# henry-yeh/DeepACO

Measured on AMD Instinct MI355X. Metric: ant-tours/sec, TSP-500 n_ants=512, higher is better.
Workload: dtype f32; 1 GPU; TSP-500 random-Euclidean, n_ants=512, 64 instances per GPU, AS update, heuristic 1/d sparsified k=50, sampler=auto -> scan_sparse; nodes=500, n_ants=512, instances_per_gpu=64, sampler=scan_sparse, parallelism=instance-sharded x1

## Files before the change

### deepaco_amd/csrc/daco_scan_sparse.hip

```cpp
#include "daco_sample_kernel.h"
#include "daco_head_rows.h"
#include "daco_tour_epilogue.h"

namespace daco {

constexpr int SP_FCMP_OGT = 2, SP_FCMP_OGE = 3, SP_FCMP_OLT = 4;

enum : uint32_t { STREAM_SPARSE = 4, STREAM_SPARSE_RETRY = 5 };

template <int N> __device__ inline float sp_row_bcast(float x) { return dpp_f<0x150 + N, 0xF, false>(x, x); }
template <int N> __device__ inline int sp_row_ror(int x) { return dpp_i<0x120 + N, 0xF, false>(x, x); }
__device__ inline float sp_row_scan(float x) {
  x = x + dpp_f<DPP_ROW_SHR(1), 0xF, true>(0.0f, x);
  x = x + dpp_f<DPP_ROW_SHR(2), 0xF, true>(0.0f, x);
  x = x + dpp_f<DPP_ROW_SHR(4), 0xF, true>(0.0f, x);
  x = x + dpp_f<DPP_ROW_SHR(8), 0xF, true>(0.0f, x);
  return x;
}
__device__ inline uint64_t sp_row_first(uint64_t m) { return m & ~((m | 0x8000800080008000ull) - 0x0001000100010001ull); }

template <bool RACE, bool VEC4, int CH>
__global__ void __launch_bounds__(256)
sparse_prepass_kernel(int B, int n, int ch, const float *tau, long tau_bs, const float *eta, long eta_bs,
                      const uint16_t *hid, float *P, char *hrow, int spl, int dead) {
  __shared__ uint32_t bm[4][32];
  const int lane = threadIdx.x & 63, wave = threadIdx.x >> 6;
  const long row = (long)blockIdx.x * 4 + wave;
  if (row >= (long)B * n) return;
  const int b = (int)(row / n), r = (int)(row - (long)b * n);
  const float *tr = tau + b * tau_bs + (long)r * n, *er = eta + b * eta_bs + (long)r * n;
  emit_head_row<RACE, CH, VEC4>(n, ch, tr, er, hid + row * (16 * spl), bm[wave], hrow + row * sp_head_row_bytes(spl), P + row * (256 * ch), spl, dead, lane);
}

template <int CH>
__global__ void __launch_bounds__(256)
sparse_prepass_ut_kernel(int B, int n, int ch, const float *tau, long tau_bs, const float *heta, float tail_c, const uint16_t *hid,
                         char *hrow, int spl, int dead) {
  __shared__ uint32_t bm[4][32];
  const int lane = threadIdx.x & 63, wave = threadIdx.x >> 6;
  const long row = (long)blockIdx.x * 4 + wave;
  if (row >= (long)B * n) return;
  const int b = (int)(row / n), r = (int)(row - (long)b * n);
  HeadUt h;
  head_ut_fetch(h, n, heta + row * (16 * spl), hid + row * (16 * spl), spl, lane);
  emit_head_row_ut<CH>(n, ch, tau + b * tau_bs + (long)r * n, tail_c, h, bm[wave], hrow + row * sp_head_row_bytes(spl), spl, dead, lane);
}

typedef uint32_t sp_u32x4 __attribute__((ext_vector_type(4)));
typedef uint32_t sp_u32x2 __attribute__((ext_vector_type(2)));
struct SpRowSrc { const float *p; };
struct SpRowUT { __amdgpu_buffer_rsrc_t t; float c; };
struct SpRowTE { __amdgpu_buffer_rsrc_t t, e; };
__device__ __forceinline__ __amdgpu_buffer_rsrc_t sp_row_rsrc(const float *row, int n) {
  return __builtin_amdgcn_make_buffer_rsrc((void *)row, 0, (int)((uint32_t)n * 4u), 0x00020000);
}
__device__ __forceinline__ int sp_lane_off(const SpRowSrc &, int lane) { return lane; }
template <class Src> __device__ __forceinline__ int sp_lane_off(const Src &, int lane) {
  int lo = lane * 16;
  asm volatile("" : "+v"(lo));
  return lo;
}
__device__ __forceinline__ float4 sp_row4(const SpRowSrc &r, int c, int lo) { return *reinterpret_cast<const float4 *>(r.p + (c * 64 + lo) * 4); }
__device__ __forceinline__ float4 sp_row4(const SpRowUT &r, int c, int lo) {
  const sp_u32x4 t = __builtin_amdgcn_raw_buffer_load_b128(r.t, lo + c * 1024, 0, 0);
  return make_float4(__uint_as_float(t.x) * r.c, __uint_as_float(t.y) * r.c, __uint_as_float(t.z) * r.c, __uint_as_float(t.w) * r.c);
}
__device__ __forceinline__ float4 sp_row4(const SpRowTE &r, int c, int lo) {
  const sp_u32x4 t = __builtin_amdgcn_raw_buffer_load_b128(r.t, lo + c * 1024, 0, 0), e = __builtin_amdgcn_raw_buffer_load_b128(r.e, lo + c * 1024, 0, 0);
  return make_float4(__uint_as_float(t.x) * __uint_as_float(e.x), __uint_as_float(t.y) * __uint_as_float(e.y),
                     __uint_as_float(t.z) * __uint_as_float(e.z), __uint_as_float(t.w) * __uint_as_float(e.w));
}

typedef const __attribute__((address_space(4))) SampleParams *sp_args_t;
template <bool UT>
__device__ __forceinline__ auto sp_row_of(const float *base, sp_args_t pa, int b, int row, int ld, int n) {
  if constexpr (UT) asm volatile("" : "+s"(pa));
  if constexpr (UT) return SpRowUT{sp_row_rsrc(pa->tau + (size_t)b * pa->tau_bs + (size_t)row * n, n), pa->tail_c};
  else return SpRowSrc{base + (size_t)row * ld};
}

template <int CHD, bool TAIL, class Src>
__device__ __forceinline__ int sparse_row_walk(const Src &rowp, const uint8_t *flg, const uint32_t *bm, int lane, float ur) {
  constexpr int NJ = CHD * 4;
  float run[16];
  float acc = 0.0f;
  uint32_t pos = 0;
  const int lo = sp_lane_off(rowp, lane);
#pragma unroll
  for (int c = 0; c < CHD; ++c) {
    const int k0 = (c * 64 + lane) * 4;
    if constexpr (std::is_same<Src, SpRowTE>::value) __builtin_amdgcn_sched_barrier(0);
    const float4 rv = sp_row4(rowp, c, lo);
    float f[4];
    if constexpr (TAIL) {
      const uint32_t w = bm[(k0 >> 5) & 31] >> (k0 & 31);
      f[0] = (w & 1u) ? 0.0f : 1.0f; f[1] = (w & 2u) ? 0.0f : 1.0f; f[2] = (w & 4u) ? 0.0f : 1.0f; f[3] = (w & 8u) ? 0.0f : 1.0f;
    } else {
      const uint32_t ff = *reinterpret_cast<const uint32_t *>(flg + k0);
      f[0] = (float)(ff & 0xFFu); f[1] = (float)((ff >> 8) & 0xFFu); f[2] = (float)((ff >> 16) & 0xFFu); f[3] = (float)(ff >> 24);
    }
    acc = __builtin_fmaf(rv.x, f[0], acc); run[4 * c + 0] = acc;
    acc = __builtin_fmaf(rv.y, f[1], acc); run[4 * c + 1] = acc;
    acc = __builtin_fmaf(rv.z, f[2], acc); run[4 * c + 2] = acc;
    acc = __builtin_fmaf(rv.w, f[3], acc); run[4 * c + 3] = acc;
    pos |= (rv.x * f[0] > 0.0f ? 1u : 0u) << (4 * c) | (rv.y * f[1] > 0.0f ? 2u : 0u) << (4 * c) |
           (rv.z * f[2] > 0.0f ? 4u : 0u) << (4 * c) | (rv.w * f[3] > 0.0f ? 8u : 0u) << (4 * c);
  }
#pragma unroll
  for (int j = NJ; j < 16; ++j) run[j] = __builtin_inff();
  const float part = acc;
  const float incl = wave_scan_add(part);
  float r = ur;
  if constexpr (!TAIL) {
    const float S = readlane_f(incl, 63);
    if (!(S > 0.0f)) return -1;
    r = ur * S;
    r = r > 0.0f ? r : 1.401298464e-45f;
  }
  uint64_t m = __ballot(incl >= r && part > 0.0f);
  int L;
  if (m == 0) {
    if constexpr (!TAIL) return -1;
    m = __ballot(part > 0.0f);
    if (m == 0) return -1;
    L = 63 - __builtin_clzll(m);
  } else {
    L = __builtin_ctzll(m);
  }
  const float excl = L ? readlane_f(incl, L - 1) : 0.0f;
  const float thr = fmaxf(r - excl, 1.401298464e-45f);
  const int cnt = count_below<NJ>(run, thr);
  int jsel = readlane_i(cnt, L);
  if (jsel >= NJ) {
    const uint32_t pl = (uint32_t)readlane_i((int)pos, L);
    jsel = pl ? 31 - __builtin_clz(pl) : 0;
  }
  return ((jsel >> 2) * 64 + L) * 4 + (jsel & 3);
}

__device__ inline float sp_at_least_denorm(float x) {
  float y;
  asm("v_max_f32 %0, 1, %1" : "=v"(y) : "v"(x));
  return y;
}

constexpr int SP_W = 352;
constexpr int SP_EW = 160;
constexpr int SP_ST_DEAD = 16 * (512 + 16) + 4 * 128 + 256;
constexpr int SP_ST_LDS = SP_ST_DEAD + 16 * SP_W * 2;
static_assert(SP_ST_LDS <= 160 * 1024 / 8 && SP_ST_DEAD % 16 == 0, "ST: eight workgroups per CU");
static_assert(SP_ST_DEAD >= 16 * SP_EW * 2 + 4 * 512 * 2, "ST: early parts and the inverse table of four ants inside the dead bytes");

static_assert(std::is_trivially_copyable<SampleParams>::value, "SampleParams is read back from the kernel-argument segment as plain bytes");
template <int CHD, bool RACE, int SPL, bool LH = false, bool ST = false, bool UT = false>
__global__ void __launch_bounds__(256, LH ? 1 : (ST ? 8 : (CHD == 2 ? (RACE ? 4 : 6) : 5)))
scan_sparse_kernel(const SampleParams p) {
  static_assert(!UT || !RACE, "the uniform-tail mode: scan draw");
  static_assert(!LH || (CHD == 2 && !RACE && SPL == 4), "the LDS-heads variant: n <= 512, scan draw, 64-slot heads");
  static_assert(!ST || (CHD == 2 && !RACE && SPL == 4 && !LH), "the split-tour variant: n <= 512, scan draw, 64-slot heads, not LH");
  constexpr int APW = 4, APB = LH ? 4 : 16;
  constexpr int LS = sp_lane_bytes(SPL);
  constexpr int LAST = SPL - 1;
  constexpr int FL = CHD * 256;
  constexpr int FLP = FL + 16;
  constexpr int FLT = FL + 2;
  constexpr uint32_t ROWB = 16u * LS;
  constexpr bool TG = CHD == 4;
  extern __shared__ __attribute__((aligned(16))) unsigned char sparse_dyn[];
  uint8_t *flag_mem = sparse_dyn;
  uint16_t *tour_mem = reinterpret_cast<uint16_t *>(sparse_dyn + (ST ? SP_ST_DEAD : APB * FLP));
  __shared__ uint32_t bm_static[TG || ST ? 1 : (LH ? 1 : 4)][32];
  uint32_t (*bm_s)[32] = TG ? reinterpret_cast<uint32_t (*)[32]>(sparse_dyn + APB * FLP + APB * 32)
                            : ST ? reinterpret_cast<uint32_t (*)[32]>(sparse_dyn + APB * FLP) : bm_static;
  unsigned char *lh_tab = sparse_dyn + APB * FLP + APB * FLT * 2;
  static_assert(!LH || ((APB * FLP + APB * FLT * 2) % 16 == 0), "LH: table aligned");
  const int lane = threadIdx.x & 63, wave = __builtin_amdgcn_readfirstlane(threadIdx.x >> 6);
  const int q = lane >> 4, s = lane & 15;
  const int w = xcd_remap(blockIdx.x, gridDim.x);
  const int bpi = (p.A + APB - 1) / APB;
  const int b = w / bpi;
  const int abase = (w - b * bpi) * APB;
  const int a0 = abase + wave * APW;
  const int n = p.n, A = p.A;
  const uint64_t iter_now = p.iter + (p.iter_dev ? *p.iter_dev : 0ull);
  const bool active = a0 < A && (!LH || wave == 0);
  const int a = a0 + q < A ? a0 + q : A - 1;
  const uint32_t gid = p.ant_gid0 + (uint32_t)(b * (p.gid_bstride ? p.gid_bstride : A) + a);
  const float *Pb = UT ? nullptr : p.P + (size_t)b * n * p.ld;
  const char *hrb = (const char *)p.hval + (size_t)b * n * ROWB;
  const __amdgpu_buffer_rsrc_t hres = __builtin_amdgcn_make_buffer_rsrc((void *)hrb, 0, (int)((uint32_t)n * ROWB), 0x00020000);
#define SP_ROW_OF(pv) sp_row_of<UT>(Pb, (sp_args_t)__builtin_amdgcn_kernarg_segment_ptr(), b, pv, p.ld, n)
  uint32_t sls = (uint32_t)s * LS;
  asm volatile("" : "+v"(sls));
  uint8_t *fl = flag_mem + (wave * APW + q) * FLP;
  uint16_t *tour = tour_mem + (wave * APW + q) * (TG ? 16 : ST ? SP_W : FLT);
  uint16_t *t16b = TG || ST ? p.tours16 + ((size_t)b * A + abase) * FL : nullptr;
  const int TE = ST ? (n > SP_W ? (n - SP_W + 15) & ~15 : 0) : 0;
  const uint32_t t16o = (uint32_t)((wave * APW + q) * FL + s);
#define SP_T(t) (TG ? ((t) & 15) : (t))
  bool infeasible = false;
  unsigned long long n_dense = 0, n_tail = 0, n_rej = 0;
  uint32_t lh_rb = 0, lh_rbsel = 0, lh_loff = 0, lh_toff = 0;
  if constexpr (LH) {
    const int kl = p.lh_kl, kmax = p.lh_kmax;
    lh_rb = (uint32_t)kl * LS;
    lh_toff = (uint32_t)(kmax / SPL) * LS + (uint32_t)(kmax % SPL) * 4u;
    lh_rbsel = s < kl ? lh_rb : 0u;
    lh_loff = s < kl ? (uint32_t)s * LS : (uint32_t)n * lh_rb;
    const char *src = hrb;
    const int l16 = threadIdx.x & 15;
    if (l16 < kl)
      for (int row0 = threadIdx.x >> 4; row0 < n; row0 += 16 * 8) {
        uint2 x[8][3];
#pragma unroll
        for (int u = 0; u < 8; ++u) {
          const int row = row0 + 16 * u;
          const uint2 *g = reinterpret_cast<const uint2 *>(src + (size_t)(row < n ? row : row0) * ROWB + l16 * LS);
          x[u][0] = g[0]; x[u][1] = g[1]; x[u][2] = g[2];
        }
#pragma unroll
        for (int u = 0; u < 8; ++u) {
          const int row = row0 + 16 * u;
          if (row < n) {
            uint2 *d = reinterpret_cast<uint2 *>(lh_tab + (uint32_t)row * lh_rb + l16 * LS);
            d[0] = x[u][0]; d[1] = x[u][1]; d[2] = x[u][2];
          }
        }
      }
    if (threadIdx.x < 4) reinterpret_cast<float *>(lh_tab + (uint32_t)n * lh_rb)[threadIdx.x] = 0.0f;
    if (threadIdx.x >= 4 && threadIdx.x < 6) reinterpret_cast<uint32_t *>(lh_tab + (uint32_t)n * lh_rb)[threadIdx.x] = (uint32_t)p.ld * 0x00010001u;
    __syncthreads();
    bool too_many = false;
    for (int row = threadIdx.x; row < n; row += 256) {
      const char *gr = src + (size_t)row * ROWB;
      const uint16_t idk = *reinterpret_cast<const uint16_t *>(gr + (kmax / SPL) * LS + SPL * 4 + (kmax % SPL) * 2);
      too_many |= idk != (uint16_t)p.ld;
      *reinterpret_cast<float *>(lh_tab + (uint32_t)row * lh_rb + lh_toff) = *reinterpret_cast<const float *>(gr + 15 * LS + LAST * 4);
    }
    if (too_many && p.flags) atomicOr(p.flags + b, 4);
    __syncthreads();
  }

  if (active) {
    {
      const uint4 ones = make_uint4(0x01010101u, 0x01010101u, 0x01010101u, 0x01010101u);
#pragma unroll
      for (int g = 0; g < FL / 256; ++g) *(uint4 *)(fl + g * 256 + s * 16) = ones;
      fl[FL + s] = 0;
    }
    int prev;
    if (p.start) prev = (int)p.start[(size_t)b * A + a];
    else if (p.fixed_start >= 0) prev = p.fixed_start;
    else {
      const u32x4 r = rng_block(p.seed, iter_now, STREAM_START, gid, 0);
      prev = (int)__umulhi(r.x, (uint32_t)n);
    }
    __builtin_amdgcn_wave_barrier();
    if (s == 0) { fl[prev] = 0; tour[0] = (uint16_t)prev; }
    asm volatile("" ::: "memory");
    __builtin_amdgcn_wave_barrier();
    u32x4 ublk = {0, 0, 0, 0};
    float ucur = 0.0f;
    for (int t0 = 0; t0 < n; t0 += 16) {
      int t = t0;
      if constexpr (ST) {
        if (t0 == TE && t0 != 0) {
          int lf = lane;
          asm volatile("" : "+v"(lf) :: "memory");
          const int qf = lf >> 4;
          const uint4 *src = reinterpret_cast<const uint4 *>(tour);
          uint4 *dst = reinterpret_cast<uint4 *>(t16b + (size_t)(wave * APW + qf) * FL);
          for (int j = lf & 15; j < (TE >> 3); j += 16) {
            const uint4 v = src[j];
            if (a0 + qf < A) dst[j] = v;
          }
          asm volatile("" ::: "memory");
          tour -= TE;
        }
      }
      if constexpr (!RACE) {
        if ((t0 & 63) == 0) ublk = rng_block(p.seed, iter_now, STREAM_SPARSE, gid, (uint32_t)(((t0 >> 6) << 4) + (15 - s)));
        ucur = u01(comp(ublk, (t0 >> 4) & 3));
        if (t0 == 0) ucur = __int_as_float(sp_row_ror<1>(__float_as_int(ucur)));
      }
      if (t0 == 0) t = 1;
      const int te = t0 + 16 < n ? t0 + 16 : n;
#ifndef DACO_SPARSE_UNROLL
#define DACO_SPARSE_UNROLL 1
#endif
#pragma unroll DACO_SPARSE_UNROLL
      for (; t < te; ++t) {
        const uint32_t off = LH ? __umul24((uint32_t)prev, lh_rbsel) + lh_loff : __umul24((uint32_t)prev, ROWB) + sls;
        float h[SPL];
        uint32_t w0, w1, w2 = 0, w3 = 0;
        if constexpr (LH) {
          const uint2 ra = *reinterpret_cast<const uint2 *>(lh_tab + off), rb_ = *reinterpret_cast<const uint2 *>(lh_tab + off + 8),
                      rc = *reinterpret_cast<const uint2 *>(lh_tab + off + 16);
          const float tv = *reinterpret_cast<const float *>(lh_tab + __umul24((uint32_t)prev, lh_rb) + lh_toff);
          h[0] = __uint_as_float(ra.x); h[1] = __uint_as_float(ra.y); h[2] = __uint_as_float(rb_.x);
          h[3] = s == 15 ? tv : __uint_as_float(rb_.y);
          w0 = rc.x; w1 = rc.y;
        } else if constexpr (SPL == 4) {
          const sp_u32x4 hvr = __builtin_amdgcn_raw_buffer_load_b128(hres, off, 0, 0);
          const sp_u32x2 hi2 = __builtin_amdgcn_raw_buffer_load_b64(hres, off + 16u, 0, 0);
          h[0] = __uint_as_float(hvr.x); h[1] = __uint_as_float(hvr.y); h[2] = __uint_as_float(hvr.z); h[3] = __uint_as_float(hvr.w);
          w0 = hi2.x; w1 = hi2.y;
        } else {
          const sp_u32x4 hva = __builtin_amdgcn_raw_buffer_load_b128(hres, off, 0, 0);
          const sp_u32x4 hvb = __builtin_amdgcn_raw_buffer_load_b128(hres, off + 16u, 0, 0);
          const sp_u32x4 hi4 = __builtin_amdgcn_raw_buffer_load_b128(hres, off + 32u, 0, 0);
          h[0] = __uint_as_float(hva.x); h[1] = __uint_as_float(hva.y); h[2] = __uint_as_float(hva.z); h[3] = __uint_as_float(hva.w);
          h[4] = __uint_as_float(hvb.x); h[5] = __uint_as_float(hvb.y); h[6] = __uint_as_float(hvb.z); h[7] = __uint_as_float(hvb.w);
          w0 = hi4.x; w1 = hi4.y; w2 = hi4.z; w3 = hi4.w;
        }
        if constexpr (SPL == 8) asm volatile("" : "+v"(w0), "+v"(w1), "+v"(w2), "+v"(w3));
#define SP_IDW(j) ((j) == 0 ? w0 : (j) == 1 ? w1 : (j) == 2 ? w2 : w3)
#define SP_ID(v) (((v) & 1) ? (int)(SP_IDW((v) >> 1) >> 16) : (int)(SP_IDW((v) >> 1) & 0xFFFFu))
        if constexpr (RACE) {
          const float rtail = sp_row_bcast<15>(h[LAST]);
          float bk = __builtin_inff();
          int bi = 0x7fffffff;
#pragma unroll
          for (int v = 0; v < SPL; ++v) {
            const int k = SP_ID(v);
            const u32x4 r4 = rng_block(p.seed, iter_now, STREAM_RACE, gid, ((uint32_t)t << 12) | (uint32_t)(k >> 2));
            const float Lk = neg_log2_1m(u01(comp(r4, k & 3)));
            const float key = fl[k] != 0 ? Lk * h[v] : __builtin_inff();
            if (prefer<false>(key, k, bk, bi)) { bk = key; bi = k; }
          }
          arg_step<false, DPP_ROW_SHR(1), 0xF>(bk, bi);
          arg_step<false, DPP_ROW_SHR(2), 0xF>(bk, bi);
          arg_step<false, DPP_ROW_SHR(4), 0xF>(bk, bi);
          arg_step<false, DPP_ROW_SHR(8), 0xF>(bk, bi);
          const float best = sp_row_bcast<15>(bk);
          int choice = __float_as_int(sp_row_bcast<15>(__int_as_float(bi)));
          const float lmin = neg_log2_1m(0x1p-24f);
          uint64_t rare = __ballot(!(best < 0.5f * lmin * rtail)) & 0x0001000100010001ull;
          while (rare) {
            const int gl = __builtin_ctzll(rare);
            rare &= rare - 1;
            const int g = gl >> 4;
            const int pv = readlane_i(prev, gl);
            const uint32_t gidg = (uint32_t)readlane_i((int)gid, gl);
            const uint8_t *flg = flag_mem + (wave * APW + g) * FLP;
            const auto rowp = SP_ROW_OF(pv);
            n_dense += a0 + g < A ? 1ull : 0ull;
            float dk = __builtin_inff();
            int di = 0x7fffffff;
#pragma unroll
            for (int c = 0; c < CHD; ++c) {
              const int k0 = (c * 64 + lane) * 4;
              const float4 pvv = sp_row4(rowp, c, sp_lane_off(rowp, lane));
              const uint32_t ff = *reinterpret_cast<const uint32_t *>(flg + k0);
              const u32x4 r4 = rng_block(p.seed, iter_now, STREAM_RACE, gidg, ((uint32_t)t << 12) | (uint32_t)(c * 64 + lane));
              const float pp[4] = {pvv.x, pvv.y, pvv.z, pvv.w};
#pragma unroll
              for (int v = 0; v < 4; ++v) {
                const float Lk = neg_log2_1m(u01(comp(r4, v)));
                const float key = ((ff >> (8 * v)) & 0xFFu) ? Lk * (1.0f / pp[v]) : __builtin_inff();
                if (key < dk) { dk = key; di = k0 + v; }
              }
            }
            const KeyIdx rr = wave_arg<false>(dk, di);
            int cg = rr.idx;
            if (!(rr.key < __builtin_inff())) { infeasible = true; cg = 0; }
            choice = q == g ? cg : choice;
          }
          if (s == 0) { fl[choice] = 0; tour[SP_T(t)] = (uint16_t)choice; }
          asm volatile("" ::: "memory");
          __builtin_amdgcn_wave_barrier();
          prev = choice;
        } else {
          float f[SPL], run[SPL];
#pragma unroll
          for (int v = 0; v < SPL; ++v) f[v] = (float)fl[SP_ID(v)];
          run[0] = __builtin_fmaf(h[0], f[0], 0.0f);
#pragma unroll
          for (int v = 1; v < SPL; ++v) run[v] = __builtin_fmaf(h[v], f[v], run[v - 1]);
          const float incl = sp_row_scan(run[LAST]);
          const float excl = dpp_f<DPP_ROW_SHR(1), 0xF, true>(0.0f, incl);
          const float r = sp_row_bcast<15>(sp_at_least_denorm(ucur * (incl + h[LAST])));
          ucur = __int_as_float(sp_row_ror<1>(__float_as_int(ucur)));

#define SP_LAST_POSITIVE(out)                                                                                     \
          do {                                                                                                    \
            int lp_ = 0;                                                                                          \
            _Pragma("unroll") for (int v = 1; v < SPL; ++v) lp_ = h[v] * f[v] > 0.0f ? v : lp_;                   \
            const uint64_t lo_ = ((uint64_t)w1 << 32) | w0, hi_ = ((uint64_t)w3 << 32) | w2;                      \
            out = (int)(((lp_ >= 4 ? hi_ : lo_) >> (16 * (lp_ & 3))) & 0xFFFFu);                                  \
          } while (0)
#define SP_HEAD_DECIDE(rr, first_out, sel_out)                                                                    \
          do {                                                                                                    \
            const float rr_ = (rr);                                                                               \
            const uint64_t m_ = __builtin_amdgcn_fcmpf(incl, rr_, SP_FCMP_OGE) & __builtin_amdgcn_fcmpf(run[LAST], 0.0f, SP_FCMP_OGT); \
            first_out = sp_row_first(m_);                                                                         \
            const float thr_ = sp_at_least_denorm(rr_ - excl);                                                    \
            bool below_[SPL];                                                                                     \
            _Pragma("unroll") for (int v = 0; v < SPL - 1; ++v) below_[v] = run[v] < thr_;                        \
            uint32_t pair_;                                                                                       \
            if constexpr (SPL == 4) pair_ = below_[1] ? w1 : w0;                                                  \
            else pair_ = below_[3] ? (below_[5] ? w3 : w2) : (below_[1] ? w1 : w0);                               \
            bool odd_ = below_[0];                                                                                \
            _Pragma("unroll") for (int v = 1; v < SPL - 1; ++v) odd_ = odd_ != below_[v];                         \
            sel_out = odd_ ? (int)(pair_ >> 16) : (int)(pair_ & 0xFFFFu);                                         \
            const uint64_t bad_ = first_out & __builtin_amdgcn_fcmpf(run[LAST], thr_, SP_FCMP_OLT);               \
            if (__builtin_expect(bad_ != 0, 0)) {                                                                 \
              int lastp_;                                                                                         \
              SP_LAST_POSITIVE(lastp_);                                                                           \
              sel_out = run[LAST] < thr_ ? lastp_ : sel_out;                                                      \
            }                                                                                                     \
          } while (0)
          int sel;
          uint64_t first;
          SP_HEAD_DECIDE(r, first, sel);


          if (__builtin_expect(__builtin_popcountll(first) != APW, 0)) {
            uint64_t any = first | (first >> 8);
            any |= any >> 4; any |= any >> 2; any |= any >> 1;
            uint64_t rare = ~any & 0x0001000100010001ull;
            while (rare) {
              const int gl = __builtin_ctzll(rare);
              rare &= rare - 1;
              const int g = gl >> 4;
              const int pv = readlane_i(prev, gl);
              const float Hg = readlane_f(incl, gl + 15);
              const float ug = readlane_f(ucur, gl), rg = readlane_f(r, gl);
              const uint32_t gidg = (uint32_t)readlane_i((int)gid, gl);
              const uint8_t *flg = flag_mem + (wave * APW + g) * FLP;
              const auto rowp = SP_ROW_OF(pv);
              int choice_g = -1;
              const unsigned long long real = a0 + g < A ? 1ull : 0ull;
              if (!(Hg > 0.0f)) {
                n_dense += real;
                choice_g = sparse_row_walk<CHD, false>(rowp, flg, nullptr, lane, ug);
              } else {
                n_tail += real;
                if (lane < 32) bm_s[wave][lane] = 0u;
                asm volatile("" ::: "memory");
                __builtin_amdgcn_wave_barrier();
                if (q == g) {
#pragma unroll
                  for (int v = 0; v < SPL; ++v) {
                    const int idl = SP_ID(v);
                    if (idl < n) atomicOr(&bm_s[wave][idl >> 5], 1u << (idl & 31));
                  }
                }
                asm volatile("" ::: "memory");
                __builtin_amdgcn_wave_barrier();
                float rp = rg - Hg;
                rp = rp > 0.0f ? rp : 1.401298464e-45f;
                const int j = sparse_row_walk<CHD, true>(rowp, flg, bm_s[wave], lane, rp);
                if (j < 0) {
                  const bool live_lane = q == g && run[LAST] > 0.0f;
                  const uint64_t ml = __ballot(live_lane);
                  if (ml != 0) {
                    const int Ll = 63 - __builtin_clzll(ml);
                    int lastp;
                    SP_LAST_POSITIVE(lastp);
                    choice_g = readlane_i(lastp, Ll);
                  }
                } else if (flg[j] != 0) {
                  choice_g = j;
                } else {
                  n_rej += real;
                  n_dense += real;
                  const u32x4 rb = rng_block(p.seed, iter_now, STREAM_SPARSE_RETRY, gidg, (uint32_t)t << 8);
                  if constexpr (UT) {
                    sp_args_t pr_ = (sp_args_t)__builtin_amdgcn_kernarg_segment_ptr();
                    asm volatile("" : "+s"(pr_));
                    const SpRowTE rowe{rowp.t, sp_row_rsrc(pr_->eta + (size_t)b * pr_->eta_bs + (size_t)pv * n, n)};
                    choice_g = sparse_row_walk<CHD, false>(rowe, flg, nullptr, lane, u01(rb.x));
                  } else {
                    choice_g = sparse_row_walk<CHD, false>(rowp, flg, nullptr, lane, u01(rb.x));
                  }
                }
              }
              if (choice_g < 0) { infeasible = true; choice_g = 0; }
              if (lane == gl) { fl[choice_g] = 0; tour[SP_T(t)] = (uint16_t)choice_g; }
            }
          }
          const bool winner = __builtin_amdgcn_inverse_ballot_w64(first);
          if (winner) { fl[sel] = 0; tour[SP_T(t)] = (uint16_t)sel; }
          asm volatile("" ::: "memory");
          prev = tour[SP_T(t)];
          asm volatile("" ::: "memory");
        }
      }
      if constexpr (TG) {
        asm volatile("" ::: "memory");
        const uint16_t wv = tour[s];
        if (a0 + q < A) t16b[t16o + (uint32_t)t0] = wv;
        asm volatile("" ::: "memory");
      }
    }
  }
#undef SP_T
#undef SP_ROW_OF
#undef SP_HEAD_DECIDE
#undef SP_LAST_POSITIVE
#undef SP_ID
#undef SP_IDW
  sp_args_t pe = (sp_args_t)__builtin_amdgcn_kernarg_segment_ptr();
  if constexpr (ST) asm volatile("" : "+s"(pe));
#define SP_E(x) (ST ? pe->x : p.x)
  if (infeasible && SP_E(flags) && lane == 0) atomicOr(SP_E(flags) + b, 1);
  if (SP_E(stats) && lane == 0 && (n_dense | n_tail | n_rej)) {
    atomicAdd(SP_E(stats) + 0, n_dense); atomicAdd(SP_E(stats) + 1, n_tail); atomicAdd(SP_E(stats) + 2, n_rej);
  }

  const int nant = A - abase < APB ? A - abase : APB;
  if constexpr (!TG) {
    uint16_t (*tour_s)[FLT] = reinterpret_cast<uint16_t (*)[FLT]>(tour_mem);
    __syncthreads();
    uint16_t (*early_s)[SP_EW] = reinterpret_cast<uint16_t (*)[SP_EW]>(sparse_dyn);
    uint16_t (*late_s)[SP_W] = reinterpret_cast<uint16_t (*)[SP_W]>(tour_mem);
    std::conditional_t<ST, TourSplit<SP_EW, SP_W>, TourRows<uint16_t>> tours;
    if constexpr (ST) tours = {&early_s[0][0], &late_s[0][0], TE};
    else tours = {&tour_s[0][0], FLT};
    if constexpr (ST) {
      if (TE > 0) {
        const int V = TE >> 3;
        for (int e = threadIdx.x; e < APB * V; e += 256) {
          const int k = e / V, j = e - k * V;
          reinterpret_cast<uint4 *>(early_s[k])[j] = reinterpret_cast<const uint4 *>(t16b + (size_t)(k < nant ? k : nant - 1) * FL)[j];
        }
        __syncthreads();
      }
    }
    if (SP_E(paths)) epi_paths<APB, !LH>(tours, SP_E(paths) + (size_t)b * n * A + abase, n, A, nant);
    if constexpr (ST) {
      if (!SP_E(paths) && SP_E(tours16)) {
        uint32_t *tb = reinterpret_cast<uint32_t *>(SP_E(tours16) + ((size_t)b * A + abase) * FL + TE);
        const int wl = (TE + SP_W < FL ? SP_W : FL - TE) / 2;
        for (int e = threadIdx.x; e < nant * (SP_W / 2); e += 256) {
          const int k = e / (SP_W / 2), j = e - k * (SP_W / 2);
          if (j < wl) tb[(size_t)k * (FL / 2) + j] = reinterpret_cast<const uint32_t *>(late_s[k])[j];
        }
      }
    } else if (!SP_E(paths) && SP_E(tours16)) {
      uint32_t *tb = reinterpret_cast<uint32_t *>(SP_E(tours16) + ((size_t)b * A + abase) * FL);
      for (int e = threadIdx.x; e < nant * (FL / 2); e += 256) {
        const int k = e / (FL / 2), j = e - k * (FL / 2);
        tb[(size_t)k * (FL / 2) + j] = reinterpret_cast<const uint32_t *>(tour_s[k])[j];
      }
    }
    if (SP_E(costs)) {
      __syncthreads();
      constexpr int DSW = ST ? 32 : 64;
      float (*dstage)[APW][DSW] = reinterpret_cast<float (*)[APW][DSW]>(LH ? lh_tab : ST ? sparse_dyn + APB * SP_EW * 2 : flag_mem);
      if (active)
        epi_tour_costs<DSW, APW>(tours, wave * APW, nant, n, SP_E(dist) + (size_t)b * SP_E(dist_bs), SP_E(dist_symmetric) != 0,
                                 &dstage[wave][0][0], SP_E(costs) + (size_t)b * A + abase);
    }
    if (SP_E(nbr)) {
      constexpr int NI = ST ? 4 : 8;
      uint16_t *inv = reinterpret_cast<uint16_t *>(LH ? lh_tab + 4096 : ST ? sparse_dyn + APB * SP_EW * 2 : flag_mem);
      static_assert(LH || ST || APB * FLP >= 8 * FL * (int)sizeof(uint16_t), "inverse table of eight ants inside the flag array");
      for (int half = 0; half < 16 / NI; ++half) {
        const int nh = nant - half * NI < NI ? nant - half * NI : NI;
        __syncthreads();
        if (nh <= 0) break;
        const int a8 = abase + half * NI;
        uint32_t *nb = SP_E(nbr_grouped) ? SP_E(nbr) + (((size_t)b * ((A + 7) >> 3) + (a8 >> 3)) * n) * 8 + (a8 & 7) : SP_E(nbr) + (size_t)b * n * A + a8;
        epi_nbr_table<NI>(tours, half * NI, inv, FL, nh, n, nb, SP_E(nbr_grouped) ? 8 : (size_t)A);
      }
    }
#undef SP_E
  } else {
    uint16_t (*tl)[FL] = reinterpret_cast<uint16_t (*)[FL]>(sparse_dyn);
    uint16_t (*inv)[FL] = reinterpret_cast<uint16_t (*)[FL]>(sparse_dyn + 8 * FL * 2);
    const int k8 = threadIdx.x & 7;
    for (int half = 0; half < 2; ++half) {
      const int nh = nant - half * 8 < 8 ? nant - half * 8 : 8;
      __syncthreads();
      if (nh <= 0) break;
      {
        constexpr int V = FL * 2 / 16;
        const uint4 *src = reinterpret_cast<const uint4 *>(t16b + (size_t)half * 8 * FL);
        for (int e = threadIdx.x; e < 8 * V; e += 256)
          if (e / V < nh) reinterpret_cast<uint4 *>(&tl[0][0])[e] = src[e];
      }
      __syncthreads();
      if (p.paths) epi_paths<8>(TourRows<uint16_t>{&tl[0][0], FL}, p.paths + (size_t)b * n * A + abase + half * 8, n, A, nh);
      if (p.costs) {
        const float *dist_b = p.dist + (size_t)b * p.dist_bs;
        float (*dstage)[2][64] = reinterpret_cast<float (*)[2][64]>(&inv[0][0]);
        const int hh = lane >> 5;
        const int mine = wave * 2 + hh;
        float cost = 0.0f;
        for (int base = 1; base < n; base += 64) {
          const int t = base + lane;
#pragma unroll
          for (int r2 = 0; r2 < 2; ++r2) {
            const uint16_t *tr = tl[wave * 2 + r2];
            dstage[wave][r2][lane] = t < n && wave * 2 + r2 < nh ? dist_b[epi_edge(tr[t], tr[t - 1], n, false)] : 0.0f;
          }
          __builtin_amdgcn_wave_barrier();
          if ((lane & 31) == 0) cost = epi_chunk_sum<64>(cost, dstage[wave][hh]);
          __builtin_amdgcn_wave_barrier();
        }
        if ((lane & 31) == 0 && mine < nh) {
          const uint16_t *tm = tl[mine];
          cost = cost + dist_b[epi_edge(tm[0], tm[n - 1], n, false)];
          p.costs[(size_t)b * A + abase + half * 8 + mine] = cost;
        }
      }
      if (p.nbr) {
        __syncthreads();
        for (int e = threadIdx.x; e < 8 * FL / 8; e += 256) ((uint4 *)&inv[0][0])[e] = make_uint4(0, 0, 0, 0);
        __syncthreads();
        const uint16_t *tk = tl[k8 < nh ? k8 : 0];
        if (k8 < nh)
          for (int t = threadIdx.x >> 3; t < n; t += 32) inv[k8][tk[t]] = (uint16_t)t;
        __syncthreads();
        const int a8 = abase + half * 8;
        uint32_t *nb = p.nbr_grouped ? p.nbr + (((size_t)b * ((A + 7) >> 3) + (a8 >> 3)) * n) * 8 + (a8 & 7) : p.nbr + (size_t)b * n * A + a8;
        const size_t nstride = p.nbr_grouped ? 8 : (size_t)A;
        if (k8 < nh)
          for (int node = threadIdx.x >> 3; node < n; node += 32) {
            const int t = inv[k8][node];
            const uint32_t pv = tk[t == 0 ? n - 1 : t - 1], nx = tk[t == n - 1 ? 0 : t + 1];
            nb[(size_t)node * nstride + k8] = pv | (nx << 16);
          }
      }
    }
  }
}

}

using namespace daco;

__global__ void __launch_bounds__(256)
pow_pair_kernel(long count_t, const float *tau, float alpha, float *tau_out, long count_e, const float *eta, float beta, float *eta_out) {
  const long i = (long)blockIdx.x * 256 + threadIdx.x;
  if (i < count_t) tau_out[i] = pw(tau[i], alpha);
  if (i < count_e) eta_out[i] = pw(eta[i], beta);
}

static bool sparse_sizes_ok(int B, int n, int A) { return B > 0 && A > 0 && n > 128 && n <= 1024; }
extern "C" size_t daco_tsp_sparse_tours_offset(int B, int n, int A) { return sparse_sizes_ok(B, n, A) ? HeadWs::tours_offset(B, n) : 0; }
extern "C" size_t daco_tsp_sparse_workspace_bytes(int B, int n, int A) { return sparse_sizes_ok(B, n, A) ? HeadWs::bytes(B, n, A) : 0; }
extern "C" size_t daco_tsp_sparse_workspace_bytes_general(int B, int n, int A) { return sparse_sizes_ok(B, n, A) ? HeadWs::bytes_general(B, n, A) : 0; }

constexpr int SP_WHOLE_TOUR_PER_CU = 6, SP_SPLIT_TOUR_PER_CU = 8;
static int sparse_split_mode = -1;
extern "C" int daco_tsp_sparse_split_tours(int mode) {
  const int old = sparse_split_mode;
  if (mode >= -1 && mode <= 1) sparse_split_mode = mode;
  return old;
}
static bool sparse_many_workgroups(long workgroups) {
  if (sparse_split_mode >= 0) return sparse_split_mode == 1;
  int dev = 0, cus = 0;
  if (hipGetDevice(&dev) != hipSuccess || hipDeviceGetAttribute(&cus, hipDeviceAttributeMultiprocessorCount, dev) != hipSuccess) { (void)hipGetLastError(); return true; }
  return workgroups > (long)SP_WHOLE_TOUR_PER_CU * cus && workgroups <= (long)SP_SPLIT_TOUR_PER_CU * cus;
}

struct SparseVariant { const void *fn; size_t lds; };
static SparseVariant sparse_variant(int ld, bool race, int spl, bool many, bool ut = false) {
#define DACO_SPARSE_LDS(C) ((C) == 2 ? 16 * ((C) * 256 + 16) + 16 * ((C) * 256 + 2) * 2 : 2 * 8 * (C) * 256 * 2)
#define DACO_SPARSE_V(C, R, S) SparseVariant{reinterpret_cast<const void *>(&scan_sparse_kernel<C, R, S>), (size_t)DACO_SPARSE_LDS(C)}
#define DACO_SPARSE_U(C, S) SparseVariant{reinterpret_cast<const void *>(&scan_sparse_kernel<C, false, S, false, false, true>), (size_t)DACO_SPARSE_LDS(C)}
  if (ut) {
    if (ld <= 512 && spl == 4 && many) return SparseVariant{reinterpret_cast<const void *>(&scan_sparse_kernel<2, false, 4, false, true, true>), (size_t)SP_ST_LDS};
    if (ld <= 512) return spl == 4 ? DACO_SPARSE_U(2, 4) : DACO_SPARSE_U(2, 8);
    return spl == 4 ? DACO_SPARSE_U(4, 4) : DACO_SPARSE_U(4, 8);
  }
#undef DACO_SPARSE_U
  if (ld <= 512 && !race && spl == 4 && many) return SparseVariant{reinterpret_cast<const void *>(&scan_sparse_kernel<2, false, 4, false, true>), (size_t)SP_ST_LDS};
  if (ld <= 512) return race ? (spl == 4 ? DACO_SPARSE_V(2, true, 4) : DACO_SPARSE_V(2, true, 8)) : (spl == 4 ? DACO_SPARSE_V(2, false, 4) : DACO_SPARSE_V(2, false, 8));
  return race ? (spl == 4 ? DACO_SPARSE_V(4, true, 4) : DACO_SPARSE_V(4, true, 8)) : (spl == 4 ? DACO_SPARSE_V(4, false, 4) : DACO_SPARSE_V(4, false, 8));
#undef DACO_SPARSE_V
#undef DACO_SPARSE_LDS
}

extern "C" int daco_tsp_sparse_resident_per_cu(int n, int head_slots, int race) {
  if (n <= 128 || n > 1024 || (head_slots != 64 && head_slots != 128)) return 0;
  const SparseVariant v = sparse_variant(HeadWs::ld_for(n), race != 0, head_slots / 16, true);
  int nb = 0;
  if (hipOccupancyMaxActiveBlocksPerMultiprocessor(&nb, v.fn, 256, v.lds) != hipSuccess) { (void)hipGetLastError(); return 0; }
  return nb;
}

extern "C" int daco_tsp_sample_heads(void *stream, int race, int heads_ready, int head_live_max, int nbr_grouped, int dist_symmetric,
                                     int B, int n, int A, const float *tau, long tau_bstride, const float *eta,
                                     long eta_bstride, float alpha, float beta, const uint16_t *head_id, int head_slots, const int64_t *start,
                                     int fixed_start, uint64_t seed, uint64_t iter, const uint64_t *iter_offset,
                                     uint32_t ant_gid0, int ant_gid_bstride, int64_t *paths, int32_t *flags, const float *dist,
                                     long dist_bstride, float *costs, uint32_t *nbr, unsigned long long *stats, void *workspace,
                                     size_t workspace_bytes, void *ev_begin, void *ev_end, const float *head_eta, float tail_c) {
  const char *const what = "daco_tsp_sample_heads";
  if (!head_eta && tail_c != 0.0f) { set_error("%s: bad argument (head_eta)", what); return DACO_E_BADARG; }
  if (B <= 0 || A <= 0 || !tau || !eta || !head_id || !workspace || (!paths && !nbr && !costs)) {
    set_error("%s: bad argument (B=%d n=%d A=%d)", what, B, n, A);
    return DACO_E_BADARG;
  }
  if (head_slots != 64 && head_slots != 128) { set_error("%s: head_slots = %d (64 or 128)", what, head_slots); return DACO_E_BADARG; }
  if (n <= 128 || n > 1024) { set_error("%s: n=%d outside 129..1024 (the dense samplers serve the other sizes)", what, n); return DACO_E_TOOLARGE; }
  if ((size_t)n * A * 8 >= ((size_t)1 << 32)) { set_error("%s: n * A too large for 32-bit offsets", what); return DACO_E_TOOLARGE; }
  if (fixed_start >= n) { set_error("%s: fixed_start %d >= n %d", what, fixed_start, n); return DACO_E_BADARG; }
  if (costs && !dist) { set_error("%s: fused costs need the distance matrix", what); return DACO_E_BADARG; }
  const size_t need = daco_tsp_sparse_workspace_bytes(B, n, A);
  if (workspace_bytes < need) { set_error("%s: workspace %zu < %zu bytes", what, workspace_bytes, need); return DACO_E_WORKSPACE; }
  hipStream_t s = (hipStream_t)stream;
  const HeadWs ws = HeadWs::carve(workspace, B, n, A);
  const int ld = ws.ld;
  const int spl = head_slots / 16;
  const bool ut = head_eta != nullptr;
  if (ut && (race || alpha != 1.0f || beta != 1.0f || !rows_vec4(n, tau, tau_bstride, eta, eta_bstride) || !(tail_c >= 0.0f))) {
    set_error("%s: the uniform-tail mode serves the scan draw with alpha = beta = 1, n %% 4 == 0, 16-byte-aligned rows of tau and eta and tail_c >= 0 (n=%d)", what, n);
    return DACO_E_BADARG;
  }
  if (alpha != 1.0f || beta != 1.0f) {
    const size_t need_g = daco_tsp_sparse_workspace_bytes_general(B, n, A);
    if (workspace_bytes < need_g) {
      set_error("%s: alpha = %g, beta = %g need daco_tsp_sparse_workspace_bytes_general() = %zu bytes of workspace (got %zu)", what, alpha, beta, need_g, workspace_bytes);
      return DACO_E_WORKSPACE;
    }
    if (heads_ready) { set_error("%s: heads_ready needs alpha = beta = 1 (daco_pheromone_update_heads forms the rows of tau itself)", what); return DACO_E_BADARG; }
    if ((tau_bstride != 0 && tau_bstride != (long)n * n) || (eta_bstride != 0 && eta_bstride != (long)n * n)) {
      set_error("%s: exponents other than 1 need dense matrices (stride n * n between instances, or 0 for a shared one)", what);
      return DACO_E_BADARG;
    }
    const long ct = (tau_bstride ? (long)B : 1L) * n * n, ce = (eta_bstride ? (long)B : 1L) * n * n;
    const long cm = ct > ce ? ct : ce;
    hipLaunchKernelGGL(pow_pair_kernel, dim3((unsigned)((cm + 255) / 256)), dim3(256), 0, s, ct, tau, alpha, ws.tau_pow, ce, eta, beta, ws.eta_pow);
    tau = ws.tau_pow; eta = ws.eta_pow;
    alpha = beta = 1.0f;
  }
  const bool vec4 = rows_vec4(n, tau, tau_bstride, eta, eta_bstride);
  if (ut && !heads_ready) {
    const dim3 pg((unsigned)(((long)B * n + 3) / 4));
    if (ld <= 512) hipLaunchKernelGGL((sparse_prepass_ut_kernel<2>), pg, dim3(256), 0, s, B, n, ld / 256, tau, tau_bstride, head_eta, tail_c, head_id, ws.hrow, spl, ld);
    else hipLaunchKernelGGL((sparse_prepass_ut_kernel<4>), pg, dim3(256), 0, s, B, n, ld / 256, tau, tau_bstride, head_eta, tail_c, head_id, ws.hrow, spl, ld);
  } else if (!heads_ready) {
    const dim3 pg((unsigned)(((long)B * n + 3) / 4));
#define DACO_PREPASS_C(R, V, C) hipLaunchKernelGGL((sparse_prepass_kernel<R, V, C>), pg, dim3(256), 0, s, B, n, ld / 256, tau, tau_bstride, eta, eta_bstride, \
                                                   head_id, ws.P, ws.hrow, spl, ld)
#define DACO_PREPASS(R, V) do { if (ld <= 512) DACO_PREPASS_C(R, V, 2); else DACO_PREPASS_C(R, V, 4); } while (0)
    if (race) { if (vec4) DACO_PREPASS(true, true); else DACO_PREPASS(true, false); }
    else { if (vec4) DACO_PREPASS(false, true); else DACO_PREPASS(false, false); }
#undef DACO_PREPASS
#undef DACO_PREPASS_C
  }
  if (const int rc = launch_status("sparse_prepass_kernel")) return rc;
  SampleParams sp = sample_params(B, n, A, ld, ld / 256, ws.P, nullptr, nullptr, seed, iter, ant_gid0, paths, nullptr, nullptr, flags);
  sp.start = start; sp.fixed_start = fixed_start;
  sp.tau = tau; sp.tau_bs = tau_bstride; sp.eta = eta; sp.eta_bs = eta_bstride; sp.tail_c = tail_c;
  sp.iter_dev = iter_offset; sp.gid_bstride = ant_gid_bstride;
  sp.dist = dist; sp.dist_bs = dist_bstride; sp.costs = costs; sp.nbr = nbr; sp.nbr_grouped = nbr_grouped ? 1 : 0; sp.dist_symmetric = dist_symmetric ? 1 : 0;
  sp.hval = (const float *)ws.hrow; sp.hid = head_id; sp.stats = stats; sp.tours16 = ws.tours16;
  if (const int rc = record_event(ev_begin, s, "ev_begin")) return rc;
  bool lh = false;
  size_t lh_lds = 0;
  if (!race && spl == 4 && ld == 512 && head_live_max > 0 && head_live_max <= 62 && (long)B * ((A + 3) / 4) <= 256) {
    const int kl = (head_live_max + 1 + 3) / 4;
    const size_t table = (size_t)n * kl * sp_lane_bytes(4) + 32;
    lh_lds = (size_t)4 * (512 + 16) + (size_t)4 * (512 + 2) * 2 + (table > 12288 + 1024 ? table : 12288 + 1024);
    lh = lh_lds + 128 <= 160 * 1024;
    sp.lh_kl = kl; sp.lh_kmax = head_live_max;
  }
  const int bpi = lh ? (A + 3) / 4 : (A + 15) / 16;
  const dim3 grid((unsigned)(B * bpi));
  if (lh) {
    const void *lh_fn = ut ? reinterpret_cast<const void *>(&scan_sparse_kernel<2, false, 4, true, false, true>) : reinterpret_cast<const void *>(&scan_sparse_kernel<2, false, 4, true>);
    if (hipFuncSetAttribute(lh_fn, hipFuncAttributeMaxDynamicSharedMemorySize,
                            160 * 1024 - 128) != hipSuccess) { set_error("%s: hipFuncSetAttribute(dynamic LDS) failed", what); return DACO_E_HIP; }
    if (ut) hipLaunchKernelGGL((scan_sparse_kernel<2, false, 4, true, false, true>), grid, dim3(256), lh_lds, s, sp);
    else hipLaunchKernelGGL((scan_sparse_kernel<2, false, 4, true>), grid, dim3(256), lh_lds, s, sp);
  } else {
    const SparseVariant v = sparse_variant(ld, race, spl, sparse_many_workgroups((long)B * bpi), ut);
    void *args[] = {&sp};
    if (hipLaunchKernel(v.fn, grid, dim3(256), args, v.lds, s) != hipSuccess) { set_error("%s: scan_sparse_kernel launch failed", what); return DACO_E_HIP; }
  }
  if (const int rc = launch_status("scan_sparse_kernel")) return rc;
  return record_event(ev_end, s, "ev_end");
}
```

Baseline: 65.92 million ant-tours/s.

## Split dense fallback out of rare loop, prefetch row loads, branchless count_below8

Ants whose head mass is zero now get their own dense loop, separated ahead of the rare tail loop. That dense loop reuses precomputed row-base descriptors and counts n_dense with a single popcount. sparse_row_walk issues all row loads up front behind a sched barrier to overlap memory latency. It also moves the positive-mask computation into the rarely taken fallback, where it reloads the row. A branchless 8-element count_below uses fcmp masks and add-with-carry inline assembly, row scaling uses packed float2 multiplies, and the stats counters shrink to 32-bit. Together these aim to cut VALU and latency in the per-step sampling path, at the cost of more registers held live and hand-written assembly that is easy to get subtly wrong.

```diff
diff --git a/deepaco_amd/csrc/daco_scan_sparse.hip b/deepaco_amd/csrc/daco_scan_sparse.hip
--- a/deepaco_amd/csrc/daco_scan_sparse.hip
+++ b/deepaco_amd/csrc/daco_scan_sparse.hip
@@ -48,6 +48,7 @@
 
 typedef uint32_t sp_u32x4 __attribute__((ext_vector_type(4)));
 typedef uint32_t sp_u32x2 __attribute__((ext_vector_type(2)));
+typedef float sp_f32x2 __attribute__((ext_vector_type(2)));
 struct SpRowSrc { const float *p; };
 struct SpRowUT { __amdgpu_buffer_rsrc_t t; float c; };
 struct SpRowTE { __amdgpu_buffer_rsrc_t t, e; };
@@ -60,11 +61,14 @@
   asm volatile("" : "+v"(lo));
   return lo;
 }
-__device__ __forceinline__ float4 sp_row4(const SpRowSrc &r, int c, int lo) { return *reinterpret_cast<const float4 *>(r.p + (c * 64 + lo) * 4); }
-__device__ __forceinline__ float4 sp_row4(const SpRowUT &r, int c, int lo) {
-  const sp_u32x4 t = __builtin_amdgcn_raw_buffer_load_b128(r.t, lo + c * 1024, 0, 0);
-  return make_float4(__uint_as_float(t.x) * r.c, __uint_as_float(t.y) * r.c, __uint_as_float(t.z) * r.c, __uint_as_float(t.w) * r.c);
-}
+__device__ __forceinline__ float4 sp_row_ld(const SpRowSrc &r, int c, int lo) { return *reinterpret_cast<const float4 *>(r.p + (c * 64 + lo) * 4); }
+__device__ __forceinline__ float4 sp_row_val(const SpRowSrc &, float4 x) { return x; }
+__device__ __forceinline__ sp_u32x4 sp_row_ld(const SpRowUT &r, int c, int lo) { return __builtin_amdgcn_raw_buffer_load_b128(r.t, lo + c * 1024, 0, 0); }
+__device__ __forceinline__ float4 sp_row_val(const SpRowUT &r, sp_u32x4 t) {
+  const sp_f32x2 lo2 = sp_f32x2{__uint_as_float(t.x), __uint_as_float(t.y)} * r.c, hi2 = sp_f32x2{__uint_as_float(t.z), __uint_as_float(t.w)} * r.c;
+  return make_float4(lo2.x, lo2.y, hi2.x, hi2.y);
+}
+template <class Src> __device__ __forceinline__ float4 sp_row4(const Src &r, int c, int lo) { return sp_row_val(r, sp_row_ld(r, c, lo)); }
 __device__ __forceinline__ float4 sp_row4(const SpRowTE &r, int c, int lo) {
   const sp_u32x4 t = __builtin_amdgcn_raw_buffer_load_b128(r.t, lo + c * 1024, 0, 0), e = __builtin_amdgcn_raw_buffer_load_b128(r.e, lo + c * 1024, 0, 0);
   return make_float4(__uint_as_float(t.x) * __uint_as_float(e.x), __uint_as_float(t.y) * __uint_as_float(e.y),
@@ -72,11 +76,36 @@
 }
 
 typedef const __attribute__((address_space(4))) SampleParams *sp_args_t;
+struct SpRowsP { const float *base; int ld; };
+struct SpRowsUT { const float *base; float c; };
+template <bool UT>
+__device__ __forceinline__ auto sp_rows_of(const float *base, sp_args_t pa, int b, int ld) {
+  if constexpr (UT) asm volatile("" : "+s"(pa));
+  if constexpr (UT) return SpRowsUT{pa->tau + (size_t)b * pa->tau_bs, pa->tail_c};
+  else return SpRowsP{base, ld};
+}
+__device__ __forceinline__ SpRowSrc sp_row_at(const SpRowsP &r, int row, int) { return SpRowSrc{r.base + (uint32_t)row * (uint32_t)r.ld}; }
+__device__ __forceinline__ SpRowUT sp_row_at(const SpRowsUT &r, int row, int n) { return SpRowUT{sp_row_rsrc(r.base + (uint32_t)row * (uint32_t)n, n), r.c}; }
 template <bool UT>
 __device__ __forceinline__ auto sp_row_of(const float *base, sp_args_t pa, int b, int row, int ld, int n) {
-  if constexpr (UT) asm volatile("" : "+s"(pa));
-  if constexpr (UT) return SpRowUT{sp_row_rsrc(pa->tau + (size_t)b * pa->tau_bs + (size_t)row * n, n), pa->tail_c};
-  else return SpRowSrc{base + (size_t)row * ld};
+  return sp_row_at(sp_rows_of<UT>(base, pa, b, ld), row, n);
+}
+
+__device__ inline int sp_add_with_carry(int x, int y, uint64_t carry) {
+  int d;
+  asm("s_nop 1\n\tv_addc_co_u32_e64 %0, vcc, %1, %2, %3" : "=v"(d) : "v"(x), "v"(y), "s"(carry) : "vcc");
+  return d;
+}
+__device__ inline int sp_count_below8(const float (&run)[16], float t) {
+  auto pick = [](uint64_t m, float a, float b) { return __builtin_amdgcn_inverse_ballot_w64(m) ? a : b; };
+  const uint64_t m2 = __builtin_amdgcn_fcmpf(run[3], t, FCMP_OLT);
+  const uint64_t m1 = __builtin_amdgcn_fcmpf(pick(m2, run[5], run[1]), t, FCMP_OLT);
+  const float e0 = pick(m1, run[2], run[0]), e1 = pick(m1, run[6], run[4]);
+  const uint64_t m0 = __builtin_amdgcn_fcmpf(pick(m2, e1, e0), t, FCMP_OLT);
+  int x = __builtin_amdgcn_inverse_ballot_w64(m2) ? 1 : 0;
+  x = sp_add_with_carry(x, x, m1);
+  x = sp_add_with_carry(x, x, m0);
+  return sp_add_with_carry(x, 0, __builtin_amdgcn_fcmpf(run[7], t, FCMP_OLT));
 }
 
 template <int CHD, bool TAIL, class Src>
@@ -84,14 +113,10 @@
   constexpr int NJ = CHD * 4;
   float run[16];
   float acc = 0.0f;
-  uint32_t pos = 0;
   const int lo = sp_lane_off(rowp, lane);
-#pragma unroll
-  for (int c = 0; c < CHD; ++c) {
+  constexpr bool TE = std::is_same<Src, SpRowTE>::value;
+  auto factors = [&](int c, float (&f)[4]) {
     const int k0 = (c * 64 + lane) * 4;
-    if constexpr (std::is_same<Src, SpRowTE>::value) __builtin_amdgcn_sched_barrier(0);
-    const float4 rv = sp_row4(rowp, c, lo);
-    float f[4];
     if constexpr (TAIL) {
       const uint32_t w = bm[(k0 >> 5) & 31] >> (k0 & 31);
       f[0] = (w & 1u) ? 0.0f : 1.0f; f[1] = (w & 2u) ? 0.0f : 1.0f; f[2] = (w & 4u) ? 0.0f : 1.0f; f[3] = (w & 8u) ? 0.0f : 1.0f;
@@ -99,12 +124,24 @@
       const uint32_t ff = *reinterpret_cast<const uint32_t *>(flg + k0);
       f[0] = (float)(ff & 0xFFu); f[1] = (float)((ff >> 8) & 0xFFu); f[2] = (float)((ff >> 16) & 0xFFu); f[3] = (float)(ff >> 24);
     }
+  };
+  typename std::conditional<std::is_same<Src, SpRowUT>::value, sp_u32x4, float4>::type raw[TE ? 1 : CHD];
+  if constexpr (!TE) {
+#pragma unroll
+    for (int c = 0; c < CHD; ++c) raw[c] = sp_row_ld(rowp, c, lo);
+    __builtin_amdgcn_sched_barrier(0);
+  }
+#pragma unroll
+  for (int c = 0; c < CHD; ++c) {
+    if constexpr (TE) __builtin_amdgcn_sched_barrier(0);
+    float4 rv;
+    if constexpr (TE) rv = sp_row4(rowp, c, lo); else rv = sp_row_val(rowp, raw[c]);
+    float f[4];
+    factors(c, f);
     acc = __builtin_fmaf(rv.x, f[0], acc); run[4 * c + 0] = acc;
     acc = __builtin_fmaf(rv.y, f[1], acc); run[4 * c + 1] = acc;
     acc = __builtin_fmaf(rv.z, f[2], acc); run[4 * c + 2] = acc;
     acc = __builtin_fmaf(rv.w, f[3], acc); run[4 * c + 3] = acc;
-    pos |= (rv.x * f[0] > 0.0f ? 1u : 0u) << (4 * c) | (rv.y * f[1] > 0.0f ? 2u : 0u) << (4 * c) |
-           (rv.z * f[2] > 0.0f ? 4u : 0u) << (4 * c) | (rv.w * f[3] > 0.0f ? 8u : 0u) << (4 * c);
   }
 #pragma unroll
   for (int j = NJ; j < 16; ++j) run[j] = __builtin_inff();
@@ -115,9 +152,9 @@
     const float S = readlane_f(incl, 63);
     if (!(S > 0.0f)) return -1;
     r = ur * S;
-    r = r > 0.0f ? r : 1.401298464e-45f;
-  }
-  uint64_t m = __ballot(incl >= r && part > 0.0f);
+    r = fmaxf(r, 1.401298464e-45f);
+  }
+  uint64_t m = __builtin_amdgcn_fcmpf(incl, r, SP_FCMP_OGE) & __builtin_amdgcn_fcmpf(part, 0.0f, SP_FCMP_OGT);
   int L;
   if (m == 0) {
     if constexpr (!TAIL) return -1;
@@ -129,9 +166,19 @@
   }
   const float excl = L ? readlane_f(incl, L - 1) : 0.0f;
   const float thr = fmaxf(r - excl, 1.401298464e-45f);
-  const int cnt = count_below<NJ>(run, thr);
+  const int cnt = NJ == 8 ? sp_count_below8(run, thr) : count_below<NJ>(run, thr);
   int jsel = readlane_i(cnt, L);
-  if (jsel >= NJ) {
+  if (__builtin_expect(jsel >= NJ, 0)) {
+    asm volatile("" ::: "memory");
+    uint32_t pos = 0;
+#pragma unroll
+    for (int c = 0; c < CHD; ++c) {
+      const float4 rv = sp_row4(rowp, c, lo);
+      float f[4];
+      factors(c, f);
+      pos |= (rv.x * f[0] > 0.0f ? 1u : 0u) << (4 * c) | (rv.y * f[1] > 0.0f ? 2u : 0u) << (4 * c) |
+             (rv.z * f[2] > 0.0f ? 4u : 0u) << (4 * c) | (rv.w * f[3] > 0.0f ? 8u : 0u) << (4 * c);
+    }
     const uint32_t pl = (uint32_t)readlane_i((int)pos, L);
     jsel = pl ? 31 - __builtin_clz(pl) : 0;
   }
@@ -199,7 +246,7 @@
   const uint32_t t16o = (uint32_t)((wave * APW + q) * FL + s);
 #define SP_T(t) (TG ? ((t) & 15) : (t))
   bool infeasible = false;
-  unsigned long long n_dense = 0, n_tail = 0, n_rej = 0;
+  unsigned n_dense = 0, n_tail = 0, n_rej = 0;
   uint32_t lh_rb = 0, lh_rbsel = 0, lh_loff = 0, lh_toff = 0;
   if constexpr (LH) {
     const int kl = p.lh_kl, kmax = p.lh_kmax;
@@ -344,7 +391,7 @@
             const uint32_t gidg = (uint32_t)readlane_i((int)gid, gl);
             const uint8_t *flg = flag_mem + (wave * APW + g) * FLP;
             const auto rowp = SP_ROW_OF(pv);
-            n_dense += a0 + g < A ? 1ull : 0ull;
+            n_dense += a0 + g < A ? 1u : 0u;
             float dk = __builtin_inff();
             int di = 0x7fffffff;
 #pragma unroll
@@ -419,61 +466,74 @@
             uint64_t any = first | (first >> 8);
             any |= any >> 4; any |= any >> 2; any |= any >> 1;
             uint64_t rare = ~any & 0x0001000100010001ull;
-            while (rare) {
+            uint64_t dense = rare & (~__builtin_amdgcn_fcmpf(incl, 0.0f, SP_FCMP_OGT) >> 15);
+            rare &= ~dense;
+            if (dense) {
+              const auto rows = sp_rows_of<UT>(Pb, (sp_args_t)__builtin_amdgcn_kernarg_segment_ptr(), b, p.ld);
+              n_dense += (unsigned)__builtin_popcountll(dense & (~0ull >> (64 - 16 * (A - a0 < APW ? A - a0 : APW))));
+              do {
+                const int gl = __builtin_ctzll(dense);
+                dense &= dense - 1;
+                const int g = gl >> 4;
+                const int pv = readlane_i(prev, gl);
+                const float ug = readlane_f(ucur, gl);
+                int choice_g = sparse_row_walk<CHD, false>(sp_row_at(rows, pv, n), flag_mem + (wave * APW + g) * FLP, nullptr, lane, ug);
+                if (choice_g < 0) { infeasible = true; choice_g = 0; }
+                if (lane == gl) { fl[choice_g] = 0; tour[SP_T(t)] = (uint16_t)choice_g; }
+              } while (dense);
+            }
+            while (__builtin_expect(rare != 0, 0)) {
               const int gl = __builtin_ctzll(rare);
               rare &= rare - 1;
+              if constexpr (SPL == 8) asm volatile("" : "+v"(w0), "+v"(w1), "+v"(w2), "+v"(w3));
+              else asm volatile("" : "+v"(w0), "+v"(w1));
               const int g = gl >> 4;
               const int pv = readlane_i(prev, gl);
               const float Hg = readlane_f(incl, gl + 15);
-              const float ug = readlane_f(ucur, gl), rg = readlane_f(r, gl);
+              const float rg = readlane_f(r, gl);
               const uint32_t gidg = (uint32_t)readlane_i((int)gid, gl);
               const uint8_t *flg = flag_mem + (wave * APW + g) * FLP;
               const auto rowp = SP_ROW_OF(pv);
               int choice_g = -1;
-              const unsigned long long real = a0 + g < A ? 1ull : 0ull;
-              if (!(Hg > 0.0f)) {
+              const unsigned real = a0 + g < A ? 1u : 0u;
+              n_tail += real;
+              if (lane < 32) bm_s[wave][lane] = 0u;
+              asm volatile("" ::: "memory");
+              __builtin_amdgcn_wave_barrier();
+              if (q == g) {
+#pragma unroll
+                for (int v = 0; v < SPL; ++v) {
+                  const int idl = SP_ID(v);
+                  if (idl < n) atomicOr(&bm_s[wave][idl >> 5], 1u << (idl & 31));
+                }
+              }
+              asm volatile("" ::: "memory");
+              __builtin_amdgcn_wave_barrier();
+              float rp = rg - Hg;
+              rp = rp > 0.0f ? rp : 1.401298464e-45f;
+              const int j = sparse_row_walk<CHD, true>(rowp, flg, bm_s[wave], lane, rp);
+              if (j < 0) {
+                const bool live_lane = q == g && run[LAST] > 0.0f;
+                const uint64_t ml = __ballot(live_lane);
+                if (ml != 0) {
+                  const int Ll = 63 - __builtin_clzll(ml);
+                  int lastp;
+                  SP_LAST_POSITIVE(lastp);
+                  choice_g = readlane_i(lastp, Ll);
+                }
+              } else if (flg[j] != 0) {
+                choice_g = j;
+              } else {
+                n_rej += real;
                 n_dense += real;
-                choice_g = sparse_row_walk<CHD, false>(rowp, flg, nullptr, lane, ug);
-              } else {
-                n_tail += real;
-                if (lane < 32) bm_s[wave][lane] = 0u;
-                asm volatile("" ::: "memory");
-                __builtin_amdgcn_wave_barrier();
-                if (q == g) {
-#pragma unroll
-                  for (int v = 0; v < SPL; ++v) {
-                    const int idl = SP_ID(v);
-                    if (idl < n) atomicOr(&bm_s[wave][idl >> 5], 1u << (idl & 31));
-                  }
-                }
-                asm volatile("" ::: "memory");
-                __builtin_amdgcn_wave_barrier();
-                float rp = rg - Hg;
-                rp = rp > 0.0f ? rp : 1.401298464e-45f;
-                const int j = sparse_row_walk<CHD, true>(rowp, flg, bm_s[wave], lane, rp);
-                if (j < 0) {
-                  const bool live_lane = q == g && run[LAST] > 0.0f;
-                  const uint64_t ml = __ballot(live_lane);
-                  if (ml != 0) {
-                    const int Ll = 63 - __builtin_clzll(ml);
-                    int lastp;
-                    SP_LAST_POSITIVE(lastp);
-                    choice_g = readlane_i(lastp, Ll);
-                  }
-                } else if (flg[j] != 0) {
-                  choice_g = j;
+                const u32x4 rb = rng_block(p.seed, iter_now, STREAM_SPARSE_RETRY, gidg, (uint32_t)t << 8);
+                if constexpr (UT) {
+                  sp_args_t pr_ = (sp_args_t)__builtin_amdgcn_kernarg_segment_ptr();
+                  asm volatile("" : "+s"(pr_));
+                  const SpRowTE rowe{rowp.t, sp_row_rsrc(pr_->eta + (size_t)b * pr_->eta_bs + (size_t)pv * n, n)};
+                  choice_g = sparse_row_walk<CHD, false>(rowe, flg, nullptr, lane, u01(rb.x));
                 } else {
-                  n_rej += real;
-                  n_dense += real;
-                  const u32x4 rb = rng_block(p.seed, iter_now, STREAM_SPARSE_RETRY, gidg, (uint32_t)t << 8);
-                  if constexpr (UT) {
-                    sp_args_t pr_ = (sp_args_t)__builtin_amdgcn_kernarg_segment_ptr();
-                    asm volatile("" : "+s"(pr_));
-                    const SpRowTE rowe{rowp.t, sp_row_rsrc(pr_->eta + (size_t)b * pr_->eta_bs + (size_t)pv * n, n)};
-                    choice_g = sparse_row_walk<CHD, false>(rowe, flg, nullptr, lane, u01(rb.x));
-                  } else {
-                    choice_g = sparse_row_walk<CHD, false>(rowp, flg, nullptr, lane, u01(rb.x));
-                  }
+                  choice_g = sparse_row_walk<CHD, false>(rowp, flg, nullptr, lane, u01(rb.x));
                 }
               }
               if (choice_g < 0) { infeasible = true; choice_g = 0; }
@@ -506,7 +566,7 @@
 #define SP_E(x) (ST ? pe->x : p.x)
   if (infeasible && SP_E(flags) && lane == 0) atomicOr(SP_E(flags) + b, 1);
   if (SP_E(stats) && lane == 0 && (n_dense | n_tail | n_rej)) {
-    atomicAdd(SP_E(stats) + 0, n_dense); atomicAdd(SP_E(stats) + 1, n_tail); atomicAdd(SP_E(stats) + 2, n_rej);
+    atomicAdd(SP_E(stats) + 0, (unsigned long long)n_dense); atomicAdd(SP_E(stats) + 1, (unsigned long long)n_tail); atomicAdd(SP_E(stats) + 2, (unsigned long long)n_rej);
   }
 
   const int nant = A - abase < APB ? A - abase : APB;
```

Result: faster. 68.98 million ant-tours/s, median of 6 (+4.6%).
